# kcat/openal-soft

Measured on AMD Instinct MI355X. Metric: mixed voices/sec @48kHz 1024-sample update, HRTF stereo; fraction of HBM roofline, higher is better.
Workload: dtype f32

## Files before the change

include/oalgpu.h:

```cpp
#ifndef OALGPU_H
#define OALGPU_H

#include <stddef.h>
#include <stdint.h>

#ifdef __cplusplus
extern "C" {
#endif
#if defined(__GNUC__)
#pragma GCC visibility push(default)
#endif

#define OALGPU_BUFFER_LINE_SIZE 1024
#define OALGPU_MAX_RESAMPLER_PADDING 48
#define OALGPU_MAX_RESAMPLER_EDGE 24
#define OALGPU_HRTF_HISTORY_LENGTH 64
#define OALGPU_HRIR_LENGTH 128
#define OALGPU_MAX_SENDS 6
#define OALGPU_MAX_OUTPUT_CHANNELS 32
#define OALGPU_MAX_AMBI_CHANNELS 25
#define OALGPU_MIXER_FRAC_BITS 16

typedef enum oalgpu_error {
    OALGPU_OK = 0,
// ... 176 lines not shown
typedef struct oalgpu_voice_pan {
    float dir[3];
    float spread;
    float dry_gain;
    float send_gain[OALGPU_MAX_SENDS];
} oalgpu_voice_pan;
int oalgpu_context_set_ambi_map(oalgpu_context *ctx, const uint8_t *index, const float *scale);
int oalgpu_slot_set_ambi_map(oalgpu_context *ctx, uint32_t slot, const uint8_t *index, const float *scale);
int oalgpu_voice_set_pan(oalgpu_context *ctx, const uint32_t *voices, const oalgpu_voice_pan *pans, size_t count);

int oalgpu_buffer_queue_link(oalgpu_context *ctx, int buffer, int next_buffer);
int oalgpu_voice_init_queue(oalgpu_context *ctx, uint32_t voice, int first_buffer, int looping, int32_t position,
    uint32_t position_frac);
int oalgpu_voice_queue_state(oalgpu_context *ctx, uint32_t voice, int32_t *current_buffer, uint32_t *buffers_done);
int oalgpu_voice_queue_unqueue(oalgpu_context *ctx, uint32_t voice, uint32_t count);

typedef int32_t (*oalgpu_callback_fn)(void *userptr, void *data, int32_t num_bytes);
int oalgpu_voice_init_callback(oalgpu_context *ctx, uint32_t voice, int fmt_type, uint32_t position_frac,
    oalgpu_callback_fn fn, void *userptr);
typedef struct oalgpu_callback_state {
    int32_t position;
    uint32_t position_frac, num_blocks, block_offset;
    int32_t stopped, play_state, has_buffer;
} oalgpu_callback_state;
int oalgpu_voice_callback_state(oalgpu_context *ctx, uint32_t voice, oalgpu_callback_state *out);

enum oalgpu_adpcm_type { OALGPU_ADPCM_IMA4 = 0, OALGPU_ADPCM_MS = 1 };
int oalgpu_buffer_register_adpcm(oalgpu_context *ctx, const void *data, int adpcm_type, uint32_t channels,
    uint32_t samples_per_block, uint32_t sample_len, uint32_t loop_start, uint32_t loop_end);

int oalgpu_voice_set_start_delay(oalgpu_context *ctx, uint32_t voice, uint32_t samples);

int oalgpu_voice_set_params(oalgpu_context *ctx, const uint32_t *voices,
    const oalgpu_voice_params *params, size_t count);
typedef struct oalgpu_param_block oalgpu_param_block;
int  oalgpu_param_block_create(oalgpu_context *ctx, const uint32_t *voices,
    const oalgpu_voice_params *params, size_t count, oalgpu_param_block **out);
int  oalgpu_param_block_apply(oalgpu_context *ctx, oalgpu_param_block *block);
int  oalgpu_mix_update_run(oalgpu_context *ctx, oalgpu_param_block *const *param_blocks, uint32_t count,
    uint32_t samples_to_do, int post_process);
void oalgpu_param_block_destroy(oalgpu_param_block *block);
int oalgpu_voice_set_state(oalgpu_context *ctx, uint32_t voice, int play_state);

int oalgpu_mix_update(oalgpu_context *ctx, uint32_t samples_to_do, int post_process);
int oalgpu_sync(oalgpu_context *ctx);
typedef struct oalgpu_resident_info {
    int32_t  enabled, failed, running, door_in_device_memory;
    uint32_t launches, updates, parks, timed_launches;
    uint64_t timed_updates;
    double   timed_kernel_ms;
    uint32_t max_updates_per_launch, pad;
    double   wait_door_us, wait_reduction_us, wait_arrival_us, wait_post_us, wait_reduced_us, wait_split_us;
    double   install_us, busy_us, top_us;
} oalgpu_resident_info;
int oalgpu_resident_stats(oalgpu_context *ctx, oalgpu_resident_info *out);
int oalgpu_resident_set_short_run(oalgpu_context *ctx, uint32_t updates);
int oalgpu_resident_set_timing(oalgpu_context *ctx, int enable);
int oalgpu_resident_set_max_updates(oalgpu_context *ctx, uint32_t max_updates);
int oalgpu_set_stream(oalgpu_context *ctx, void *hip_stream);

int oalgpu_read_dry(oalgpu_context *ctx, float *out);
int oalgpu_read_wet(oalgpu_context *ctx, uint32_t slot, float *out);
int oalgpu_read_hrtf_accum(oalgpu_context *ctx, float *out);
int oalgpu_set_bformat_decoder(oalgpu_context *ctx, uint32_t num_out, const float *coeffs_hf,
    const float *coeffs_lf, float xover_norm);
enum oalgpu_output_type {
    OALGPU_OUT_I8 = 0, OALGPU_OUT_U8, OALGPU_OUT_I16, OALGPU_OUT_U16, OALGPU_OUT_I32, OALGPU_OUT_U32, OALGPU_OUT_F32
};
int oalgpu_set_output(oalgpu_context *ctx, int sample_type, float dither_depth, uint32_t dither_seed);
int oalgpu_read_output(oalgpu_context *ctx, void *out, uint32_t samples_to_do, uint32_t frame_step);
enum {
    OALGPU_LIMITER_AUTO_KNEE = 1u << 0, OALGPU_LIMITER_AUTO_ATTACK = 1u << 1, OALGPU_LIMITER_AUTO_RELEASE = 1u << 2,
    OALGPU_LIMITER_AUTO_POST_GAIN = 1u << 3, OALGPU_LIMITER_AUTO_DECLIP = 1u << 4
};
typedef struct oalgpu_limiter_params {
    uint32_t num_channels;
    float sample_rate;
    uint32_t auto_flags;
    float look_ahead_time, hold_time, pre_gain_db, post_gain_db, threshold_db, ratio, knee_db, attack_time, release_time;
} oalgpu_limiter_params;
int oalgpu_limiter_device_params(uint32_t sample_rate, int sample_type, float dither_depth, oalgpu_limiter_params *out);
uint32_t oalgpu_limiter_look_ahead(const oalgpu_limiter_params *params);
int oalgpu_set_output_limiter(oalgpu_context *ctx, const oalgpu_limiter_params *params);
enum oalgpu_uhj_quality { OALGPU_UHJ_IIR = 0, OALGPU_UHJ_FIR256, OALGPU_UHJ_FIR512 };
uint32_t oalgpu_uhj_encoder_delay(int quality);
int oalgpu_set_uhj_encoder(oalgpu_context *ctx, int quality);
enum oalgpu_tsme_quality { OALGPU_TSME_IIR = 0, OALGPU_TSME_FIR256, OALGPU_TSME_FIR512 };
uint32_t oalgpu_tsme_encoder_delay(int quality);
int oalgpu_set_tsme_encoder(oalgpu_context *ctx, int quality);
enum { OALGPU_BS2B_LOW = 1, OALGPU_BS2B_MIDDLE, OALGPU_BS2B_HIGH,
       OALGPU_BS2B_LOW_EASY, OALGPU_BS2B_MIDDLE_EASY, OALGPU_BS2B_HIGH_EASY };
int oalgpu_crossfeed_constants(int level, uint32_t sample_rate, float out[5]);
int oalgpu_set_crossfeed(oalgpu_context *ctx, int level, uint32_t left, uint32_t right);
typedef struct oalgpu_stabilizer_params {
    uint32_t left, right, center;
    float    xover_norm;
} oalgpu_stabilizer_params;
int oalgpu_front_stabilizer_constants(float xover_norm, float *out);
int oalgpu_set_front_stabilizer(oalgpu_context *ctx, const oalgpu_stabilizer_params *params);
int oalgpu_distance_comp_from_distances(uint32_t sample_rate, const float *distances, uint32_t n,
                                        uint32_t *delays, float *gains);
int oalgpu_set_distance_comp(oalgpu_context *ctx, uint32_t n, const uint32_t *delays, const float *gains);

int oalgpu_bus_device_ptr(oalgpu_context *ctx, void **ptr, size_t *nfloats, void **hip_stream);
int oalgpu_mix_voices(oalgpu_context *ctx, uint32_t samples_to_do);
int oalgpu_post_process(oalgpu_context *ctx, uint32_t samples_to_do);
// ... 188 lines not shown
```

openal-soft_amd/csrc/api.hip:

```cpp
#include "api_context.hpp"
namespace oalgpu {

thread_local std::string gLastError;

int Fail(int code, const std::string &msg)
{
    gLastError = msg;
    return code;
}

void ParkResidentContexts(int device);

int UseDevice(int device)
{
    int count = 0;
    if(hipGetDeviceCount(&count) != hipSuccess || count <= 0)
        return Fail(OALGPU_ERR_NO_DEVICE, "no HIP device available (the product has no CPU path)");
    if(device < 0 || device >= count) return Fail(OALGPU_ERR_INVALID, "device ordinal out of range");
    HIP_TRY(hipSetDevice(device));
    ParkResidentContexts(device);
    return OALGPU_OK;
}

}
// ... 927 lines not shown

int oalgpu_slot_set_effect(oalgpu_context *c, uint32_t slot, oalgpu_effect *fx)
{
    if(!c || slot >= c->L.numSlots) return Fail(OALGPU_ERR_INVALID, "oalgpu_slot_set_effect: bad slot");
    if(fx && (EffectOutLines(fx) > c->L.numDry + c->L.numReal || EffectInChannels(fx) > c->L.wetChannels))
        return Fail(OALGPU_ERR_INVALID, "oalgpu_slot_set_effect: the effect's lines do not fit the context's buses");
    if(int rc = oalgpu_sync(c)) return rc;
    c->slotEffect[slot] = fx;
    return OALGPU_OK;
}

int oalgpu_slot_set_reverb(oalgpu_context *c, uint32_t slot, oalgpu_reverb *rev)
{
    if(!c || slot >= c->L.numSlots) return Fail(OALGPU_ERR_INVALID, "oalgpu_slot_set_reverb: bad slot");
    if(rev && c->L.wetChannels < 4)
        return Fail(OALGPU_ERR_INVALID, "oalgpu_slot_set_reverb: the reverb reads a 4-line B-Format wet bus");
    if(rev && ReverbOutLines(rev) > c->L.numDry)
        return Fail(OALGPU_ERR_INVALID, "oalgpu_slot_set_reverb: the effect mixes into more lines than the context has dry lines");
    if(int rc = oalgpu_sync(c)) return rc;
    if(rev) { if(int rc = oalgpu_reverb_set_math_mode(rev, c->exact ? OALGPU_MATH_EXACT : OALGPU_MATH_FAST)) return rc; }
    c->slotReverb[slot] = rev;
    return RebalanceWaveGroups(c);
}

const char *oalgpu_voice_kernel_name(oalgpu_context *c)
{
    if(!c) return "";
    if(c->useWave) return WaveKernelName(c->L);
    return c->exact ? "VoiceMixKernel<true, LINES>" : "VoiceMixKernel<false, LINES>";
}

int oalgpu_resident_stats(oalgpu_context *c, oalgpu_resident_info *out)
{
    if(!c || !out) return Fail(OALGPU_ERR_INVALID, "null argument");
    auto &R = c->res;
    uint32_t w[kRcCount * 16] = {};
    if(R.ready && !R.running)
    {
        if(int rc = UseDevice(c->desc.device)) return rc;
        HIP_TRY(hipMemcpy(w, R.counters.p, sizeof(w), hipMemcpyDeviceToHost));
    }
    std::lock_guard<std::mutex> g(gResLock);
    out->enabled = R.enabled ? 1 : 0; out->failed = R.failed ? 1 : 0; out->running = R.running ? 1 : 0;
    out->door_in_device_memory = R.doorInBar ? 1 : 0;
    out->launches = R.launches; out->updates = R.next; out->parks = uint32_t(R.parks);
    out->timed_launches = uint32_t(R.kernelLaunches); out->timed_updates = R.kernelUpdates; out->timed_kernel_ms = R.kernelMs;
    out->max_updates_per_launch = R.maxUpdates; out->pad = 0;
    const double tick = 0.01, groups = double(std::max<uint32_t>((c->L.numGroups + 127u) / 128u, 1u));
    out->wait_door_us = w[16 * kRcWaitDoor] * tick / groups; out->wait_reduction_us = w[16 * kRcWaitRed] * tick / groups;
    out->wait_arrival_us = w[16 * kRcWaitArrive] * tick; out->wait_post_us = w[16 * kRcWaitPost] * tick;
    out->wait_reduced_us = w[16 * kRcWaitRedDone] * tick; out->wait_split_us = w[16 * kRcWaitSplit] * tick;
    out->install_us = w[16 * kRcInstall] * tick / groups; out->busy_us = w[16 * kRcBusy] * tick / groups;
    out->top_us = w[16 * kRcTop] * tick / groups;
    return OALGPU_OK;
}

int oalgpu_resident_set_short_run(oalgpu_context *c, uint32_t updates)
{
    if(!c) return Fail(OALGPU_ERR_INVALID, "null argument");
    if(int rc = UseCtx(c)) return rc;
    c->res.shortRun = updates;
    c->res.shortRuns = 0; c->res.cooldown = 0;
    return OALGPU_OK;
}

int oalgpu_resident_set_timing(oalgpu_context *c, int enable)
{
    if(!c) return Fail(OALGPU_ERR_INVALID, "null argument");
    if(int rc = UseCtx(c)) return rc;
    c->res.timeLaunches = enable != 0;
    return OALGPU_OK;
}

int oalgpu_resident_set_max_updates(oalgpu_context *c, uint32_t max_updates)
{
    if(!c || max_updates == 0 || max_updates > 0x10000000u) return Fail(OALGPU_ERR_INVALID, "oalgpu_resident_set_max_updates: 1 .. 2^28");
    if(int rc = UseCtx(c)) return rc;
    c->res.maxUpdates = max_updates;
    return OALGPU_OK;
}

int oalgpu_set_carry_accum(oalgpu_context *c, int enable)
{
    if(int rc = BeginSetter(c, "oalgpu_set_carry_accum")) return rc;
    c->carryAccum = enable != 0;
    return OALGPU_OK;
}
```

openal-soft_amd/csrc/kernels.hpp:

```cpp
#pragma once
#include <hip/hip_runtime.h>
#include <stdint.h>

#include "dev_hrtf.hpp"
#include "dev_mix.hpp"
#include "dev_resample.hpp"
#include "dev_voice.hpp"
#include "../host/limiter_params.hpp"
#include "../host/uhj_params.hpp"
#include "../host/stabilizer_params.hpp"
#include "../host/crossfeed_params.hpp"

namespace oalgpu {

enum VoiceFlagBits : uint32_t {
    kFlagFading = 1u << 0,
    kFlagHasHrtf = 1u << 1,
    kFlagDirectFilter = 1u << 2,
    kFlagHrtfDirty = 1u << 3,
    kFlagAmbiScale = 1u << 4,
    kFlagNfc = 1u << 5,
    kFlagQueue = 1u << 7,
    kFlagDelayed = 1u << 6,
    kFlagSendFilterShift = 8
// ... 124 lines not shown
            | (r.keepHrtf ? uint32_t(kFlagHrtfDirty) : 0u));
        ctl.flags = keep | (r.flags & ~(kFlagFading | kFlagHasHrtf | kFlagHrtfDirty | kFlagAmbiScale | kFlagNfc | kFlagDelayed | kFlagQueue))
            | (L.hrtf ? (kFlagHasHrtf | (r.keepHrtf ? 0u : uint32_t(kFlagHrtfDirty))) : 0u);
        for(int i = 0; i < 6; ++i) ctl.sendSlot[i] = (uint32_t(i) < L.numSends) ? r.sendSlot[i] : -1;
        if(L.hrtf && !r.keepHrtf)
        {
            ctl.hrtfTgtDelay[0] = r.hrtfDelay[0]; ctl.hrtfTgtDelay[1] = r.hrtfDelay[1];
            ctl.hrtfTgtGain = r.hrtfGain;
        }
    }
    if(lane == 1) BiquadSetTarget(L.dfilt[size_t{v} * 2 + 0].f, r.dirLp);
    if(lane == 2) BiquadSetTarget(L.dfilt[size_t{v} * 2 + 1].f, r.dirHp);
    if(lane >= 8 && lane < 8 + 2 * L.numSends)
    {
        const uint32_t i = (lane - 8) >> 1, hp = (lane - 8) & 1u;
        BiquadSetTarget(L.sfilt[(size_t{v} * L.numSends + i) * 2 + hp].f, hp ? r.sendHp[i] : r.sendLp[i]);
    }
    if(L.hrtf) { if(!r.keepHrtf) ApplyHrtfTargetWave(L, v, r.hrtfIdx, r.hrtfW, r.hrtfPass, lane); }
    else if(lane < L.numDry)
        L.gainTgt[size_t{v} * L.numDry + lane] = r.dryGains[lane];
    for(uint32_t k = lane; k < L.numSends * L.wetChannels; k += 64)
        L.sendTgt[size_t{v} * L.numSends * L.wetChannels + k] = r.sendGains[k / L.wetChannels][k % L.wetChannels];
}

struct VoiceInitRecord { uint32_t voice; int32_t buffer, looping, position; uint32_t positionFrac; int32_t queue; };

constexpr uint32_t kResidentSets = 4;
constexpr uint32_t kResidentSlots = 16;
constexpr uint32_t kResidentDepth = 8;
constexpr unsigned long long kResidentWatchdogTicks = 200000000ull;

struct ResidentSlot { unsigned long long recs, map, rows; uint32_t samples, pad; };
struct alignas(64) ResidentDoor {
    uint32_t seq;
    uint32_t exitSeq[4];
    uint32_t pad[11];
    ResidentSlot slot[kResidentSlots];
};
enum ResidentCounter : uint32_t {
    kRcArrive0 = 0,
    kRcRedRead = 4,
    kRcRedDone = 5,
    kRcPostDone = 6,
    kRcStarted = 7,
    kRcWaitDoor = 8,
    kRcWaitRed = 9,
    kRcWaitArrive = 10,
    kRcWaitPost = 11,
    kRcWaitRedDone = 12,
    kRcWaitSplit = 13,
    kRcInstall = 14,
    kRcBusy = 15,
    kRcTop = 16,
    kRcCount = 17
};
enum ResidentHostFlag : uint32_t { kRhResident = 0, kRhError = 1, kRhProgress = 2,
    kRhFault = 3,
    kRhCount = 4 };
struct ResidentArgs {
    const ResidentDoor *door;
    uint32_t *counters;
    uint32_t *hostFlags;
    float *partBase;
    uint32_t setStride;
    uint32_t base, endSeq;
    uint32_t redPerUpdate;
    uint32_t startedTarget, launchId;
};

void LaunchResample(hipStream_t s, bool exact, const ResampleSpec &spec, const float *src, uint32_t frac,
    uint32_t increment, float *dst, uint32_t n);
void LaunchMix(hipStream_t s, const float *in, uint32_t n, float *out, uint32_t nlines, float *cur,
    const float *tgt, uint32_t counter, uint32_t outpos);
void LaunchMixHrtf(hipStream_t s, bool exact, const float *in, float *accum, uint32_t irsize, const float *coeffs,
    uint32_t dL, uint32_t dR, float gain, float step, const float *oldcoeffs, uint32_t odL, uint32_t odR,
    float oldgain, int blend, uint32_t n);
void LaunchMixDirectHrtf(hipStream_t s, bool exact, float *left, float *right, const float *in, uint32_t nch,
    float *accum, SplitterState *splitters, const float *hfscales, const float *chanCoeffs, uint32_t irsize,
    uint32_t n, float *temp);
void LaunchBiquadDual(hipStream_t s, BiquadState *f0, BiquadState *f1, const float *src, float *dst, uint32_t n);
void LaunchGetCoeffs(hipStream_t s, const HrtfStoreDev &st, const float *dirs, uint32_t count, float *coeffs,
    uint32_t *delays);

void LaunchPostDirectHrtfFast(hipStream_t s, float *left, float *right, const float *in, uint32_t nch, float *accum,
    SplitterState *splitters, const float *hfscales, const float *chanCoeffs, uint32_t irsize, uint32_t n, float *temp,
    hipEvent_t evDone = nullptr);

inline uint32_t ReducePostReduceGroups(const DeviceLayout &L) { return uint32_t((BusFloats(L) + 63u) / 64u); }
void LaunchReducePostFused(hipStream_t s, const DeviceLayout &L, const float *carry, float *left, float *right, const float *in, uint32_t nch,
    const float *accIn, float *carryOut, const SplitterState *spIn, SplitterState *spOut, const float *hfscales, const float *chanCoeffs,
    uint32_t irsize, uint32_t n, float *xf, uint32_t *arrived, uint32_t epoch, const float runPower[4], hipEvent_t evDone,
    float *hostOut, uint32_t *hostFlag, uint32_t hostSeq, uint32_t *outArrived, uint32_t outTarget, uint32_t *reduced, uint32_t reducedEpoch);
void LaunchPostDirectHrtfFused(hipStream_t s, float *left, float *right, const float *in, uint32_t nch, const float *accIn, float *carryOut,
    const SplitterState *spIn, SplitterState *spOut, const float *hfscales, const float *chanCoeffs, uint32_t irsize, uint32_t n,
    float *xf, uint32_t *arrived, uint32_t epoch, const float runPower[4], hipEvent_t evDone = nullptr,
    float *hostOut = nullptr, uint32_t *hostFlag = nullptr, uint32_t hostSeq = 0, uint32_t *outArrived = nullptr, uint32_t outTarget = 0);
void LaunchBusReduceResident(hipStream_t s, const DeviceLayout &L, const float *carry, uint32_t *counters, uint32_t *hostFlags, uint32_t set,
    uint32_t arriveTarget, uint32_t postDoneTarget);
uint32_t PostResidentFirGroups();
void LaunchPostResident(hipStream_t s, float *left, float *right, const float *in, uint32_t nch, const float *accIn, float *carryOut,
    const SplitterState *spIn, SplitterState *spOut, const float *hfscales, const float *chanCoeffs, uint32_t irsize, uint32_t n,
    float *xf, uint32_t *arrived, uint32_t epoch, const float runPower[4], hipEvent_t evDone, float *hostOut, uint32_t *hostFlag, uint32_t hostSeq,
    uint32_t *counters, uint32_t *hostFlags, uint32_t redDoneTarget, uint32_t postDoneTarget, uint32_t progressValue);

void LaunchBFormatDecode(hipStream_t s, bool exact, float *out, const float *lines, SplitterState *states, float *bands,
    const float *gainsHf, const float *gainsLf, uint32_t nin, uint32_t nout, uint32_t n);
void LaunchDither(hipStream_t s, float *lines, uint32_t nlines, uint32_t n, float quantScale, uint32_t seed);
// ... 155 lines not shown
```

openal-soft_amd/csrc/voice_wave16.hip:

```cpp
#define OALGPU_WAVE_NO_LAUNCHER
#include "voice_wave.hip"

#pragma clang fp contract(off)

namespace oalgpu {
namespace {

constexpr int kW16Outs = kLine / 64;

constexpr int kW16Rd = 1184;
constexpr int kW16Rd2 = kMaxEdge + kPre * 64 + 8;
constexpr int kW16Area = kResampleDataSize + kLine;
static_assert(kW16Rd % 64 == 32 && kW16Rd >= kMaxPad + kPre * 64 + 8, "rd2 sits half the banks away from rd");
static_assert(kW16Rd + kW16Rd2 <= kW16Area, "the twice-parked window fits");
static_assert(kResampleDataSize >= kLine + 64, "a send's filter scan parks the unfiltered samples in the window's area");
constexpr int kW16DumpF2 = 64 * 17 + 68;
static_assert(kW16DumpF2 * 2 <= kW16Area, "the dump fits");
struct W16PhaseB {
    uint32_t xh[2][kXhDw];
    uint32_t hr[2][kHrDw];
    uint32_t hro[2][kHrDw];
    float in0[2 * kHist];
};
static_assert(sizeof(W16PhaseB) <= size_t(kW16Area) * 4, "phase B fits the area (nothing of it is written before the sample line is back in registers)");
// ... 104 lines not shown
            A[s][c] = __builtin_bit_cast(h8, q);
        }
#pragma unroll
    for(int T = 0; T < TILES; ++T)
    {
        __builtin_amdgcn_sched_barrier(0);
        const uint32_t j = (T == 4 && i > 3u) ? 3u : i;
        h8 B[2][3];
#pragma unroll
        for(int s = 0; s < 2; ++s)
        {
            const u4 *p = reinterpret_cast<const u4*>(xh[s]) + 32 * T + 2u * j + g;
#pragma unroll
            for(int c = 0; c < 3; ++c) B[s][c] = __builtin_bit_cast(h8, p[4 * c]);
        }
        f4 ta = {0.0f, 0.0f, 0.0f, 0.0f}, tb = ta, tc = ta;
#pragma unroll
        for(int c = 0; c < 3; ++c)
        {
            ta = __builtin_amdgcn_mfma_f32_16x16x32_f16(A[1][c], B[0][c], ta, 0, 0, 0);
            tb = __builtin_amdgcn_mfma_f32_16x16x32_f16(A[0][c], B[1][c], tb, 0, 0, 0);
            tc = __builtin_amdgcn_mfma_f32_16x16x32_f16(A[0][c], B[0][c], tc, 0, 0, 0);
        }
        f4 sum = __builtin_elementwise_fma((ta + tb) + tc, vinv, acc[T]);
        asm volatile("" : "+v"(sum));
        if(!LOW8 || i < 8u) acc[T] = sum;
        __builtin_amdgcn_sched_barrier(0);
    }
}

__device__ __forceinline__ float W16ReadLaneF(float v, int l)
{ return __builtin_bit_cast(float, __builtin_amdgcn_readlane(__builtin_bit_cast(int, v), l)); }

__device__ __forceinline__ float W16StageResponse(uint32_t (&hr)[2][kHrDw], float h, uint32_t lane)
{
    float sh, inv;
    HalfScale(WaveMaxBits(__builtin_bit_cast(uint32_t, __builtin_fabsf(h))), sh, inv);
    uint32_t hi, lo;
    SplitHalf2(h * sh, 0.0f, hi, lo);
    uint32_t *hz32 = &hr[0][0];
    for(uint32_t k = lane; k < uint32_t(2 * kHrDw); k += 64) hz32[k] = 0u;
    uint16_t *hz = reinterpret_cast<uint16_t*>(&hr[0][0]);
    const uint32_t u = 80u - lane;
    hz[0 * kHrHalves + u] = uint16_t(hi); hz[1 * kHrHalves + u] = uint16_t(lo);
    return __builtin_bit_cast(float, __builtin_amdgcn_readfirstlane(__builtin_bit_cast(int, inv)));
}

__device__ __forceinline__ uint32_t W16VoiceOf(uint32_t group, uint32_t wave, uint32_t waves)
{
    const uint32_t a = wave >> 2, b = wave & 3u;
    return group * waves + 4u * a + ((a + b) & 3u);
}

struct Next16 { const ParamRecord *recs; const int32_t *map; const float *rows; ResidentArgs res; };
struct W16Sends {
    BiquadSlot *sfilt; const float *sendTgt; float *sendCur; float *streams; uint32_t *lineGains;
    uint32_t numSends, wetCh, lineStride, spv;
};

template<bool PROF, int WAVES, bool SENDS = false, bool RES = false>
__global__ void OALGPU_SINGLE_DS_OPS __launch_bounds__(WAVES * 64) VoiceWave16Kernel(WaveArgsHrtf L, uint32_t samplesToDo, Next16 next, WaveProf prof, W16Sends S)
{
    unsigned long long tEntry = 0;
    if constexpr (PROF) tEntry = __builtin_readcyclecounter();
    constexpr uint32_t kW16Waves = uint32_t(WAVES), kW16Threads = uint32_t(WAVES) * 64u;
    __shared__ W16Wg<WAVES> sm;
    const uint32_t t = threadIdx.x;
    uint32_t lane = t & 63u;
    const uint32_t wave = __builtin_amdgcn_readfirstlane(t >> 6);
    const uint32_t group = blockIdx.x;
    const uint32_t irStride = L.irStride;
    uint32_t N = samplesToDo;
    W16Lds &w = sm.w[wave];
    asm volatile("; argument block resident" :: "s"(L.tables), "s"(L.buffers), "s"(L.ctl), "s"(L.prev), "s"(L.dfilt), "s"(L.hrtfOld),
        "s"(L.hrtfTgt), "s"(L.hist), "s"(L.ambi), "s"(L.startDelay), "s"(L.queueDone), "s"(L.partHrtf), "s"(L.hrirs),
        "s"(next.recs), "s"(next.map), "s"(L.numVoices), "s"(L.irStride), "s"(L.pad), "s"(samplesToDo));

    const uint32_t vRaw = W16VoiceOf(group, wave, kW16Waves);
    const bool haveVoice = vRaw < L.numVoices;
    const uint32_t lastVoice = L.numVoices - 1u;
    const uint32_t v = haveVoice ? vRaw : lastVoice;
    const uint32_t keyVoice = group * uint32_t(kW16Waves);

    uint32_t upd = 0u, updBase = 0u;
    if constexpr (RES)
    {
        const ResidentArgs &RA = next.res;
        upd = updBase = RA.base;
        if(t == 0)
        {
            const uint32_t old = __hip_atomic_fetch_add(RA.counters + 16u * kRcStarted, 1u, __ATOMIC_RELAXED, __HIP_MEMORY_SCOPE_AGENT);
            if(old + 1u == RA.startedTarget)
                __hip_atomic_store(RA.hostFlags + 16u * kRhResident, RA.launchId, __ATOMIC_RELAXED, __HIP_MEMORY_SCOPE_SYSTEM);
        }
    }
    for(;;)
    {
    uint32_t tU = threadIdx.x;
    if constexpr (RES) { asm volatile("" : "+v"(tU)); lane = tU & 63u; }
    const uint32_t t = tU;
    if constexpr (RES)
    {
        const ResidentArgs &RA = next.res;
        if(t == 0)
        {
            const unsigned long long tTop = __builtin_amdgcn_s_memrealtime();
            uint32_t go = 0u, fault = 0u;
            unsigned long long recs = 0ull, map = 0ull, rowsP = 0ull;
            uint32_t smp = 0u;
            if(upd != RA.endSeq)
            {
                const ResidentDoor *door = RA.door;
                const uint32_t *exitp = &door->exitSeq[RA.launchId & 3u];
                const uint32_t *rr = RA.counters + 16u * kRcRedRead;
                const bool needRed = int32_t(upd - kResidentSets) >= 0;
                const uint32_t want = (upd - kResidentSets + 1u) * RA.redPerUpdate;
                unsigned long long t0 = 0ull;
                uint32_t waitedFor = 0u;
                for(uint32_t spins = 0;; ++spins)
                {
                    const uint32_t ex = ResLoadSys(exitp), sq = ResLoadSys(&door->seq), rd = needRed ? ResLoadDev(rr) : want;
                    if(int32_t(ex - upd) <= 0) break;
                    const bool rung = int32_t(sq - upd) > 0, redOk = int32_t(rd - want) >= 0;
                    if(rung && redOk) { go = 1u; break; }
                    if(spins == 0u) { t0 = __builtin_amdgcn_s_memrealtime(); waitedFor = rung ? 2u : 1u; }
                    else if((spins & 15u) == 15u && __builtin_amdgcn_s_memrealtime() - t0 > kResidentWatchdogTicks)
                    {
                        fault = 1u;
                        uint32_t *fi = RA.hostFlags + 16u * kRhFault;
                        fi[0] = upd; fi[1] = sq; fi[2] = ex; fi[3] = rd; fi[4] = want; fi[5] = group; fi[6] = RA.launchId;
                        fi[7] = uint32_t(__builtin_amdgcn_s_memrealtime() - t0);
                        break;
                    }
                    if(spins < 32u) __builtin_amdgcn_s_sleep(2); else __builtin_amdgcn_s_sleep(24);
                }
                if(waitedFor && (group & 127u) == 0u)
                    __hip_atomic_fetch_add(RA.counters + 16u * (waitedFor == 1u ? kRcWaitDoor : kRcWaitRed), uint32_t(__builtin_amdgcn_s_memrealtime() - t0),
                        __ATOMIC_RELAXED, __HIP_MEMORY_SCOPE_AGENT);
                if(go)
                {
                    const ResidentSlot *sl = &door->slot[upd % kResidentSlots];
                    recs = ResLoadSys(&sl->recs); map = ResLoadSys(&sl->map); rowsP = ResLoadSys(&sl->rows); smp = ResLoadSys(&sl->samples);
                }
            }
            if(fault) __hip_atomic_store(RA.hostFlags + 16u * kRhError, 1u, __ATOMIC_RELAXED, __HIP_MEMORY_SCOPE_SYSTEM);
            if((group & 127u) == 0u)
                __hip_atomic_fetch_add(RA.counters + 16u * kRcTop, uint32_t(__builtin_amdgcn_s_memrealtime() - tTop), __ATOMIC_RELAXED, __HIP_MEMORY_SCOPE_AGENT);
            sm.res[0] = go; sm.res[1] = smp;
// ... 26 lines not shown
    auto stamp = [&](int slot)
    {
        if constexpr (PROF) { if(prof.times && haveVoice && (t & 63u) == 0u) prof.times[size_t{v} * 8 + slot] = __builtin_readcyclecounter(); }
    };
    if constexpr (PROF) { if(prof.times && haveVoice && (t & 63u) == 0u) prof.times[size_t{v} * 8 + 0] = tEntry; }
    auto stamp2 = [&](int slot)
    {
        if constexpr (PROF) { if(prof.times && haveVoice && (t & 63u) == 0u) prof.times[size_t{L.numVoices} * 8 + size_t{v} * 8 + slot] = __builtin_readcyclecounter(); }
    };
    const VoiceHead head = LoadHeadScalar(L.ctl + v);
    const BufferItem buf = LoadCtlBufferScalar(L.ctl + v);
    const VoiceTail tail = LoadTailScalar(L.ctl + v);
    asm volatile("" ::: "memory");
    const VoiceHead headK = LoadHeadScalar(L.ctl + (keyVoice < L.numVoices ? keyVoice : lastVoice));
    asm volatile("" ::: "memory");
    const int psK = headK.playState, kK = headK.rsKind;
    const uint32_t mK = kK == 2 ? 4u : headK.rsM, lK = kK == 2 ? 1u : headK.rsL, offK = headK.rsFilterOffset;

    const bool eligK = keyVoice < L.numVoices && (kK == 2 || (kK == 3 && (mK == 12 || mK == 24)))
        && (psK == OALGPU_VOICE_PLAYING || psK == OALGPU_VOICE_STOPPING);
    bool stageRows = true;
    if constexpr (RES) { if(upd != updBase) stageRows = !(eligK && sm.tabKey == offK * 8u + uint32_t(kK) && sm.tabM == mK); }
    if constexpr (RES) __syncthreads();
    if(eligK && stageRows)
    {
        typedef const __attribute__((address_space(1))) void *gvoidp;
        typedef __attribute__((address_space(3))) void *lvoidp;
        const float *src = L.tables + offK + size_t{lane >> 1} * (2u * mK) + (lane & 1u);
        for(uint32_t pp = wave; pp < mK / 2u; pp += uint32_t(kW16Waves))
        {
            __builtin_amdgcn_global_load_lds((gvoidp)(src + 2u * pp), (lvoidp)&sm.tabF[32u * pp], 4, 0, 0);
            __builtin_amdgcn_global_load_lds((gvoidp)(src + mK + 2u * pp), (lvoidp)&sm.tabP[32u * pp], 4, 0, 0);
        }
        if(t == 0) { sm.tabKey = offK * 8u + uint32_t(kK); sm.tabM = mK; sm.tabL = lK; }
    }

    const int vstate = head.playState;
    const bool mixes = haveVoice && (vstate == OALGPU_VOICE_PLAYING || vstate == OALGPU_VOICE_STOPPING);
    const bool playing = haveVoice && vstate == OALGPU_VOICE_PLAYING;
    bool active = mixes && head.step >= 1u;
    const bool dirty = (head.flags & kFlagHrtfDirty) != 0;
    SrcPlan plan = PlanSource(head, N);
    bool looping = false;
    if(head.curBuffer >= 0)
    {
        looping = head.loopBuffer >= 0 && ((head.flags & kFlagQueue) || !(head.position >= 0 && uint32_t(head.position) >= buf.loopEnd));
        plan.prefetch = plan.prefetch && GatherCovers(plan.bsrc, buf, looping, uint32_t(head.position));
    }
    if(head.flags & (kFlagDelayed | kFlagQueue)) plan.prefetch = false;
    const uint32_t sM = head.rsKind == 2 ? 4u : head.rsM, sL = head.rsKind == 2 ? 1u : head.rsL;
    const bool regPath = active && plan.prefetch && eligK && (head.rsKind == 2 || head.rsKind == 3)
        && head.rsFilterOffset * 8u + uint32_t(head.rsKind) == offK * 8u + uint32_t(kK) && sM == mK
        && !(head.step == kFracOne && head.positionFrac == 0u);
    float pre[kPre];
#pragma unroll
    for(int i = 0; i < kPre; ++i) pre[i] = 0.0f;
    float prevv = 0.0f;
    if(regPath)
    {
        GatherStatic(pre, plan.bsrc, buf, looping, uint32_t(head.position), lane);
        prevv = (lane < kMaxPad) ? L.prev[size_t{v} * kMaxPad + lane] : 0.0f;
    }

    if(!eligK)
    {
        if(wave == 0)
        {
            const uint32_t cand = keyVoice + lane;
            bool eligible = false;
            uint32_t off = 0, m = 0, l = 0;
            int kind = 0;
            if(lane < uint32_t(kW16Waves) && cand < L.numVoices)
            {
                const VoiceCtl &c = L.ctl[cand];
                kind = c.rsKind; off = c.rsFilterOffset; m = c.rsM; l = c.rsL;
                if(kind == 2) { m = 4; l = 1; }
                eligible = (kind == 2 || (kind == 3 && (m == 12 || m == 24)))
                    && (c.playState == OALGPU_VOICE_PLAYING || c.playState == OALGPU_VOICE_STOPPING);
            }
            const unsigned long long mask = __ballot(eligible);
            if(mask)
            {
                const int firstLane = __ffsll((long long)mask) - 1;
                const uint32_t key = uint32_t(__shfl(int(off * 8u + uint32_t(kind)), firstLane));
                const uint32_t fm = uint32_t(__shfl(int(m), firstLane)), fl = uint32_t(__shfl(int(l), firstLane));
                if(lane == 0) { sm.tabKey = key; sm.tabM = fm; sm.tabL = fl; }
            }
            else if(lane == 0) { sm.tabKey = 0xffffffffu; sm.tabM = 0; sm.tabL = 0; }
        }
        __syncthreads();
        const uint32_t key = sm.tabKey, m = sm.tabM;
        if(key != 0xffffffffu)
        {
            const float *filter = L.tables + (key >> 3);
            for(uint32_t idx = t; idx < (m / 2u) * 32u; idx += uint32_t(kW16Threads))
            {
                const uint32_t p = idx >> 5, pi = idx & 31u;
                const float *row = filter + pi * 2u * m;
                sm.tabF[idx] = f2{row[2u * p], row[2u * p + 1u]};
                sm.tabP[idx] = f2{row[m + 2u * p], row[m + 2u * p + 1u]};
            }
        }
    }
    if(regPath)
    {
        const bool isShort = buf.fmt == OALGPU_FMT_SHORT;
        if(lane < kMaxPad) { w.a.rd[lane] = prevv; if(lane) w.a.rd2[lane - 1u] = prevv; }
#pragma unroll
        for(int i = 0; i < kPre; ++i)
        {
            const float sv = GatherDecode(pre[i], isShort);
            w.a.rd[kMaxEdge + lane + 64u * uint32_t(i)] = sv;
            w.a.rd2[kMaxEdge - 1u + lane + 64u * uint32_t(i)] = sv;
        }
    }
    asm volatile("s_waitcnt vmcnt(0)" ::: "memory");
    __syncthreads();
    stamp(7);
    __builtin_amdgcn_s_setprio(2);

    uint32_t outPos = 0;
    if(mixes && !active && !playing && lane == 0) L.ctl[v].playState = OALGPU_VOICE_STOPPED;
    if(active && (head.flags & kFlagDelayed))
    {
        const uint32_t d = L.startDelay[v];
        if(!playing)
        {
            if(lane == 0) { L.ctl[v].playState = OALGPU_VOICE_STOPPED; L.ctl[v].flags = head.flags & ~kFlagDelayed; L.startDelay[v] = 0u; }
            active = false;
        }
        else if(d >= N) { if(lane == 0) L.startDelay[v] = d - N; active = false; }
        else
        {
            outPos = d;
            if(lane == 0) L.startDelay[v] = 0u;
            for(uint32_t k = lane; k < outPos; k += 64) w.g.smp[k] = 0.0f;
        }
    }

    f4 accM[2][5];
#pragma unroll
    for(int e = 0; e < 2; ++e)
#pragma unroll
        for(int b = 0; b < 5; ++b) accM[e][b] = f4{0.0f, 0.0f, 0.0f, 0.0f};

    uint32_t counter = 0, fademix = 0, todo = 0;
    float endGain = 0.0f, gainAfterBlend = 0.0f;
    float fstv = 0.0f, histv = 0.0f;
    f2 hT = {0.0f, 0.0f};
    int32_t bufferItem = head.curBuffer;
    if constexpr (SENDS)
    {
        if(haveVoice && !active && lane < S.spv)
            S.lineGains[(size_t{v} * S.spv + lane) * LineBlockDwords(S.lineStride) + 3u * S.lineStride] = 0u;
    }
    if(active)
    {
        float outs[kW16Outs];
        if(regPath)
        {
            WaveSync();
            const float *rdb = w.a.rd + (kMaxEdge - sL), *rd2b = w.a.rd2 + (kMaxEdge - sL);
            const uint32_t rdbIndex = uint32_t(kMaxEdge) - sL;
            if(sM == 24u) ResampleRingRegs<24, true>(sm.tabF, sm.tabP, rdb, head.positionFrac, head.step, N, outs, lane, rd2b, rdbIndex);
            else if(sM == 12u) ResampleRingRegs<12, true>(sm.tabF, sm.tabP, rdb, head.positionFrac, head.step, N, outs, lane, rd2b, rdbIndex);
            else ResampleRingRegs<4, false>(sm.tabF, sm.tabP, rdb, head.positionFrac, head.step, N, outs, lane, nullptr, 0u);
            asm volatile("" : "+v"(lane));
            if(playing)
            {
                const uint32_t srcOffset = uint32_t((uint64_t{N} * head.step + head.positionFrac) >> kFracBits);
                if(lane < kMaxPad) L.prev[size_t{v} * kMaxPad + lane] = w.a.rd[srcOffset + lane];
            }
        }
        else
        {
            W16GenView gv{w.g.rd, w.g.smp - kHist, nullptr, w.best, w.pad};
            LoadResampledWave<true, false>(sm, gv, L, v, lane, head, playing, N - outPos, N - outPos, bufferItem, looping,
                SrcPlan{false, plan.bdst, plan.bsrc}, outPos);
            asm volatile("" : "+v"(lane));
            WaveSync();
#pragma unroll
            for(int j = 0; j < kW16Outs; ++j) outs[j] = w.g.smp[lane + 64u * uint32_t(j)];
        }
        if(N < uint32_t(kLine))
        {
#pragma unroll
            for(int j = 0; j < kW16Outs; ++j) if(lane + 64u * uint32_t(j) >= N) outs[j] = 0.0f;
        }
        stamp(1);
        __builtin_amdgcn_s_setprio(1);
        fstv = (lane < 32u) ? reinterpret_cast<const float*>(L.dfilt + size_t{v} * 2)[lane] : 0.0f;
        histv = L.hist[size_t{v} * kHist + lane];
// ... 229 lines not shown
                __builtin_fabsf(endGain));
            HalfScale(__builtin_bit_cast(uint32_t, mxw * gmax), sx, invX);
            invX = __builtin_bit_cast(float, __builtin_amdgcn_readfirstlane(__builtin_bit_cast(int, invX)));
            sx = __builtin_bit_cast(float, __builtin_amdgcn_readfirstlane(__builtin_bit_cast(int, sx)));
        }
        const float step64 = mainStep * 64.0f * sx;
        auto buildEar = [&](uint32_t d, auto fullTag)
        {
            constexpr bool FULL = decltype(fullTag)::value;
            if(lane < 32u) { w.b.xh[0][lane] = 0u; w.b.xh[1][lane] = 0u; }
            for(uint32_t dw = 32u + (N >> 1) + lane; dw < uint32_t(kXhDw); dw += 64u) { w.b.xh[0][dw] = 0u; w.b.xh[1][dw] = 0u; }
            WaveSync();
            uint16_t *xz = reinterpret_cast<uint16_t*>(&w.b.xh[0][0]) + 64u + lane + d;
            if(lane < d)
            {
                const float headP = (lane < N) ? w.b.in0[kHist - d + lane] * gainAt(lane, true) : 0.0f;
                uint32_t hi, lo;
                SplitHalf2(headP * sx, 0.0f, hi, lo);
                uint16_t *xh0 = reinterpret_cast<uint16_t*>(&w.b.xh[0][0]) + 64u + lane;
                xh0[0] = uint16_t(hi); xh0[kXhHalves] = uint16_t(lo);
            }
            const uint32_t i00 = lane + d;
            const float g0s = gainAt(i00, true) * sx;
            const float gls = __builtin_fmaf(mainStep, float(i00), gbase) * sx;
#pragma unroll
            for(int j = 0; j < kW16Outs; j += 2)
            {
                const float ga = (j == 0) ? g0s : __builtin_fmaf(step64, float(j), gls);
                const float gb = __builtin_fmaf(step64, float(j + 1), gls);
                float p0 = outs[j] * ga, p1 = outs[j + 1] * gb;
                if(!FULL || j + 2 == kW16Outs)
                {
                    if(i00 + 64u * uint32_t(j) >= N) p0 = 0.0f;
                    if(i00 + 64u * uint32_t(j + 1) >= N) p1 = 0.0f;
                }
                uint32_t hi, lo;
                SplitHalf2(p0, p1, hi, lo);
                xz[64 * j] = uint16_t(hi); xz[kXhHalves + 64 * j] = uint16_t(lo);
                xz[64 * (j + 1)] = uint16_t(hi >> 16); xz[kXhHalves + 64 * (j + 1)] = uint16_t(lo >> 16);
            }
        };

#pragma unroll
        for(int e = 0; e < 2; ++e)
        {
            const uint32_t d = tail.tgtDelay[e];
            if(N == uint32_t(kLine)) buildEar(d, std::true_type{}); else buildEar(d, std::false_type{});
            uint16_t *xz = reinterpret_cast<uint16_t*>(&w.b.xh[0][0]);
            if(e == 0) stamp2(1);
            const float invH = W16StageResponse(w.b.hr, e == 0 ? hT.x : hT.y, lane);
            WaveSync();
            if(e == 0) stamp2(2);
            FirMfmaEar<5, false>(accM[e], w.b.xh, w.b.hr, invX * invH, lane);
            if(e == 0) stamp2(3);
            if(oldPass)
            {
                const uint32_t od = tail.oldDelay[e];
                float xo = 0.0f;
                if(lane < fademix) xo = w.b.in0[kHist - od + lane] * (oldStep * float(fademix - lane));
                float sxo, invXo;
                HalfScale(WaveMaxBits(__builtin_bit_cast(uint32_t, __builtin_fabsf(xo))), sxo, invXo);
                invXo = __builtin_bit_cast(float, __builtin_amdgcn_readfirstlane(__builtin_bit_cast(int, invXo)));
                uint32_t hi, lo;
                SplitHalf2(xo * sxo, 0.0f, hi, lo);
                WaveSync();
                xz[0 * kXhHalves + 64u + lane] = uint16_t(hi); xz[1 * kXhHalves + 64u + lane] = uint16_t(lo);
                if(lane < 40u) { w.b.xh[0][64u + lane] = 0u; w.b.xh[1][64u + lane] = 0u; }
                const float invHO = W16StageResponse(w.b.hro, e == 0 ? hO.x : hO.y, lane);
                WaveSync();
                FirMfmaEar<1, true>(accM[e], w.b.xh, w.b.hro, invXo * invHO, lane);
            }
            WaveSync();
            stamp(3 + e);
        }
    }

    if(active)
    {
        if(dirty && (counter == 0 || fademix))
        {
            if(lane < irStride) reinterpret_cast<f2*>(L.hrtfOld + size_t{v} * irStride * 2)[lane] = hT;
        }
        if(lane == 0)
        {
            VoiceCtl &c = L.ctl[v];
            if(counter == 0 || fademix) { c.hrtfOldDelay[0] = tail.tgtDelay[0]; c.hrtfOldDelay[1] = tail.tgtDelay[1]; }
            c.hrtfOldGain = todo ? endGain : gainAfterBlend;
            uint32_t flags = (head.flags | kFlagFading) & ~kFlagDelayed;
            if(counter == 0 || fademix) flags &= ~kFlagHrtfDirty;
            c.flags = flags;
            if(!playing) c.playState = OALGPU_VOICE_STOPPED;
            else
            {
                int32_t bufPosInt = head.position;
                uint32_t bufPosFrac = head.positionFrac + head.step * (N - outPos);
                const uint32_t samplesDone = bufPosFrac >> kFracBits;
                bufPosInt = AddSat(bufPosInt, int32_t(samplesDone));
                bufPosFrac &= kFracMask;
                if(bufferItem >= 0 && bufPosInt > 0 && (head.flags & kFlagQueue))
                {
                    uint32_t buffersDone = 0;
                    const int32_t before = bufferItem;
                    AdvanceQueue(L.buffers, bufferItem, head.loopBuffer, bufPosInt, buffersDone);
                    if(buffersDone) L.queueDone[v] += buffersDone;
                    if(bufferItem >= 0 && bufferItem != before) c.buf = L.buffers[bufferItem];
                }
// ... 151 lines not shown
```

openal-soft_amd/oalgpu/__init__.py:

```python
import ctypes as C
import os

import numpy as np

PKG_DIR = os.path.dirname(os.path.dirname(os.path.abspath(__file__)))
LIB_PATH = os.path.join(PKG_DIR, "liboalgpu.so")

BUFFER_LINE = 1024
MAX_PAD = 48
HRTF_HIST = 64
HRIR_LEN = 128
MAX_SENDS = 6
(OUT_I8, OUT_U8, OUT_I16, OUT_U16, OUT_I32, OUT_U32, OUT_F32) = range(7)
MAX_OUT = 32
MAX_AMBI = 25
MATH_EXACT, MATH_FAST = 0, 1
(RS_POINT, RS_LINEAR, RS_SPLINE, RS_GAUSSIAN, RS_FAST_BSINC12, RS_BSINC12, RS_FAST_BSINC24,
 RS_BSINC24, RS_FAST_BSINC48, RS_BSINC48) = range(10)
FMT_UBYTE, FMT_SHORT, FMT_INT, FMT_FLOAT, FMT_DOUBLE, FMT_MULAW, FMT_ALAW = range(7)
FMT_DTYPES = {FMT_UBYTE: np.uint8, FMT_SHORT: np.int16, FMT_INT: np.int32, FMT_FLOAT: np.float32,
              FMT_DOUBLE: np.float64, FMT_MULAW: np.uint8, FMT_ALAW: np.uint8}
VOICE_STOPPED, VOICE_PLAYING, VOICE_STOPPING, VOICE_PENDING = range(4)

f32p = C.POINTER(C.c_float)
# ... 681 lines not shown
    def set_front_stabilizer(self, left, right=None, center=None, xover_norm=5000.0 / 48000.0):
        lib.oalgpu_set_front_stabilizer.argtypes = [C.c_void_p, C.POINTER(StabilizerParams)]
        if left is None:
            check(lib.oalgpu_set_front_stabilizer(self.h, None), "oalgpu_set_front_stabilizer")
            return
        params = StabilizerParams(left, right, center, xover_norm)
        check(lib.oalgpu_set_front_stabilizer(self.h, C.byref(params)), "oalgpu_set_front_stabilizer")

    def set_distance_comp(self, delays, gains=None):
        u32p = C.POINTER(C.c_uint32)
        lib.oalgpu_set_distance_comp.argtypes = [C.c_void_p, C.c_uint32, u32p, f32p]
        if delays is None:
            check(lib.oalgpu_set_distance_comp(self.h, 0, None, None), "oalgpu_set_distance_comp")
            return
        d = np.ascontiguousarray(delays, np.uint32)
        g = np.ascontiguousarray(gains, np.float32)
        assert d.ndim == 1 and d.shape == g.shape
        check(lib.oalgpu_set_distance_comp(self.h, d.size, d.ctypes.data_as(u32p), _fp(g)), "oalgpu_set_distance_comp")

    def read_output(self, samples_to_do=BUFFER_LINE, frame_step=2):
        lib.oalgpu_read_output.argtypes = [C.c_void_p, C.c_void_p, C.c_uint32, C.c_uint32]
        dt = [np.int8, np.uint8, np.int16, np.uint16, np.int32, np.uint32, np.float32][getattr(self, "_out_type", 6)]
        out = np.zeros(samples_to_do * frame_step, dt)
        check(lib.oalgpu_read_output(self.h, out.ctypes.data_as(C.c_void_p), samples_to_do, frame_step), "oalgpu_read_output")
        return out

    def set_slot_convolution(self, slot, conv):
        lib.oalgpu_slot_set_convolution.argtypes = [C.c_void_p, C.c_uint32, C.c_void_p]
        check(lib.oalgpu_slot_set_convolution(self.h, slot, conv.h if conv is not None else None))

    def set_slot_effect(self, slot, fx):
        lib.oalgpu_slot_set_effect.argtypes = [C.c_void_p, C.c_uint32, C.c_void_p]
        check(lib.oalgpu_slot_set_effect(self.h, slot, fx.h if fx is not None else None), "oalgpu_slot_set_effect")

    def set_slot_reverb(self, slot, rev):
        lib.oalgpu_slot_set_reverb.argtypes = [C.c_void_p, C.c_uint32, C.c_void_p]
        check(lib.oalgpu_slot_set_reverb(self.h, slot, rev.h if rev is not None else None))

    def mix(self, samples_to_do=BUFFER_LINE, post_process=False):
        check(lib.oalgpu_mix_update(self.h, samples_to_do, 1 if post_process else 0),
              "oalgpu_mix_update")

    def sync(self):
        check(lib.oalgpu_sync(self.h), "oalgpu_sync")

    def resident_stats(self):
        class Info(C.Structure):
            _fields_ = [("enabled", C.c_int32), ("failed", C.c_int32), ("running", C.c_int32), ("door_in_device_memory", C.c_int32),
                        ("launches", C.c_uint32), ("updates", C.c_uint32), ("parks", C.c_uint32), ("timed_launches", C.c_uint32),
                        ("timed_updates", C.c_uint64), ("timed_kernel_ms", C.c_double),
                        ("max_updates_per_launch", C.c_uint32), ("pad", C.c_uint32),
                        ("wait_door_us", C.c_double), ("wait_reduction_us", C.c_double), ("wait_arrival_us", C.c_double),
                        ("wait_post_us", C.c_double), ("wait_reduced_us", C.c_double), ("wait_split_us", C.c_double),
                        ("install_us", C.c_double), ("busy_us", C.c_double), ("top_us", C.c_double)]
        info = Info()
        lib.oalgpu_resident_stats.argtypes = [C.c_void_p, C.POINTER(Info)]
        check(lib.oalgpu_resident_stats(self.h, C.byref(info)), "oalgpu_resident_stats")
        return {k: getattr(info, k) for k, _ in Info._fields_ if k != "pad"}

    def resident_set_short_run(self, updates):
        lib.oalgpu_resident_set_short_run.argtypes = [C.c_void_p, C.c_uint32]
        check(lib.oalgpu_resident_set_short_run(self.h, updates), "oalgpu_resident_set_short_run")

    def resident_set_timing(self, on):
        lib.oalgpu_resident_set_timing.argtypes = [C.c_void_p, C.c_int]
        check(lib.oalgpu_resident_set_timing(self.h, 1 if on else 0), "oalgpu_resident_set_timing")

    def resident_set_max_updates(self, n):
        lib.oalgpu_resident_set_max_updates.argtypes = [C.c_void_p, C.c_uint32]
        check(lib.oalgpu_resident_set_max_updates(self.h, n), "oalgpu_resident_set_max_updates")

    def dry(self):
        n = self.desc.num_dry_channels + self.desc.num_real_channels
        out = np.zeros((n, BUFFER_LINE), np.float32)
        check(lib.oalgpu_read_dry(self.h, _fp(out)), "oalgpu_read_dry")
        return out

    def wet(self, slot):
        out = np.zeros((self.desc.wet_channels, BUFFER_LINE), np.float32)
        check(lib.oalgpu_read_wet(self.h, slot, _fp(out)), "oalgpu_read_wet")
        return out

    def hrtf_accum(self):
        out = np.zeros((BUFFER_LINE + HRIR_LEN, 2), np.float32)
        check(lib.oalgpu_read_hrtf_accum(self.h, _fp(out)), "oalgpu_read_hrtf_accum")
        return out

    def voice_state(self, voice):
        st = VoiceState()
        check(lib.oalgpu_voice_readback(self.h, voice, C.byref(st)), "oalgpu_voice_readback")
        return st

    def bus_device_ptr(self):
        p, n, s = C.c_void_p(), C.c_size_t(), C.c_void_p()
        check(lib.oalgpu_bus_device_ptr(self.h, C.byref(p), C.byref(n), C.byref(s)))
        return p.value, n.value, s.value

    def voice_kernel_name(self):
        lib.oalgpu_voice_kernel_name.restype = C.c_char_p
        lib.oalgpu_voice_kernel_name.argtypes = [C.c_void_p]
        return lib.oalgpu_voice_kernel_name(self.h).decode()

    def set_timing(self, enable=True):
        check(lib.oalgpu_set_timing(self.h, 1 if enable else 0))

    def last_update_ms(self):
        a, b = C.c_float(), C.c_float()
# ... 234 lines not shown
```

Baseline: 114.6 million.

## Prefetch next update's source window during HRTF FIR in resident kernel

In the resident (persistent) kernel, the register-held source window (pre[]) and the resampler history are now gathered for the next update while the current update's second-ear MFMA FIR runs. A per-lane key over the buffer, position and loop state validates the prefetched data at the next iteration. On a match the gather at update start is skipped, otherwise it falls back to the normal gather. A timing counter (window_us) is added to the stats. The cost is extra registers kept live across iterations, which may reduce occupancy, and wasted loads whenever the prediction misses.

```diff
diff --git a/include/oalgpu.h b/include/oalgpu.h
--- a/include/oalgpu.h
+++ b/include/oalgpu.h
@@ -252,6 +252,7 @@
     uint32_t max_updates_per_launch, pad;
     double   wait_door_us, wait_reduction_us, wait_arrival_us, wait_post_us, wait_reduced_us, wait_split_us;
     double   install_us, busy_us, top_us;
+    double   window_us;
 } oalgpu_resident_info;
 int oalgpu_resident_stats(oalgpu_context *ctx, oalgpu_resident_info *out);
 int oalgpu_resident_set_short_run(oalgpu_context *ctx, uint32_t updates);
diff --git a/openal-soft_amd/csrc/api.hip b/openal-soft_amd/csrc/api.hip
--- a/openal-soft_amd/csrc/api.hip
+++ b/openal-soft_amd/csrc/api.hip
@@ -1003,6 +1003,7 @@
     out->wait_reduced_us = w[16 * kRcWaitRedDone] * tick; out->wait_split_us = w[16 * kRcWaitSplit] * tick;
     out->install_us = w[16 * kRcInstall] * tick / groups; out->busy_us = w[16 * kRcBusy] * tick / groups;
     out->top_us = w[16 * kRcTop] * tick / groups;
+    out->window_us = w[16 * kRcWindow] * tick / groups;
     return OALGPU_OK;
 }
 
diff --git a/openal-soft_amd/csrc/kernels.hpp b/openal-soft_amd/csrc/kernels.hpp
--- a/openal-soft_amd/csrc/kernels.hpp
+++ b/openal-soft_amd/csrc/kernels.hpp
@@ -200,7 +200,8 @@
     kRcInstall = 14,
     kRcBusy = 15,
     kRcTop = 16,
-    kRcCount = 17
+    kRcWindow = 17,
+    kRcCount = 18
 };
 enum ResidentHostFlag : uint32_t { kRhResident = 0, kRhError = 1, kRhProgress = 2,
     kRhFault = 3,
diff --git a/openal-soft_amd/csrc/voice_wave16.hip b/openal-soft_amd/csrc/voice_wave16.hip
--- a/openal-soft_amd/csrc/voice_wave16.hip
+++ b/openal-soft_amd/csrc/voice_wave16.hip
@@ -180,6 +180,33 @@
     return group * waves + 4u * a + ((a + b) & 3u);
 }
 
+constexpr uint32_t kW16NoWindow = 0xffffffffu;
+__device__ __forceinline__ uint32_t W16WindowKey(const BufferItem &b, int32_t curBuffer, uint32_t position, bool looping, uint32_t lane)
+{
+    const uint64_t d = uint64_t(uintptr_t(b.data));
+    uint32_t k = 0u;
+    k = lane == 0u ? uint32_t(d) : k;
+    k = lane == 1u ? uint32_t(d >> 32) : k;
+    k = lane == 2u ? uint32_t(b.fmt) : k;
+    k = lane == 3u ? b.frameStep : k;
+    k = lane == 4u ? b.sampleLen : k;
+    k = lane == 5u ? b.loopStart : k;
+    k = lane == 6u ? b.loopEnd : k;
+    k = lane == 7u ? uint32_t(b.next) : k;
+    k = lane == 8u ? uint32_t(curBuffer) : k;
+    k = lane == 9u ? position : k;
+    k = lane == 10u ? (looping ? 1u : 0u) : k;
+    return k;
+}
+__device__ __forceinline__ uint32_t W16WindowCount(const BufferItem &b, bool looping, uint32_t position)
+{
+    const uint32_t whole = uint32_t(kPre) * 64u;
+    if(!looping) return whole;
+    if(position >= b.loopEnd) return 0u;
+    const uint64_t reach = uint64_t{b.loopEnd - position} + (b.loopEnd - b.loopStart);
+    return reach < whole ? uint32_t(reach) : whole;
+}
+
 struct Next16 { const ParamRecord *recs; const int32_t *map; const float *rows; ResidentArgs res; };
 struct W16Sends {
     BiquadSlot *sfilt; const float *sendTgt; float *sendCur; float *streams; uint32_t *lineGains;
@@ -222,6 +249,14 @@
                 __hip_atomic_store(RA.hostFlags + 16u * kRhResident, RA.launchId, __ATOMIC_RELAXED, __HIP_MEMORY_SCOPE_SYSTEM);
         }
     }
+    float pre[kPre];
+    float prePrev = 0.0f;
+    uint32_t preKey = kW16NoWindow;
+    if constexpr (RES)
+    {
+#pragma unroll
+        for(int i = 0; i < kPre; ++i) pre[i] = 0.0f;
+    }
     for(;;)
     {
     uint32_t tU = threadIdx.x;
@@ -354,15 +389,28 @@
     const bool regPath = active && plan.prefetch && eligK && (head.rsKind == 2 || head.rsKind == 3)
         && head.rsFilterOffset * 8u + uint32_t(head.rsKind) == offK * 8u + uint32_t(kK) && sM == mK
         && !(head.step == kFracOne && head.positionFrac == 0u);
-    float pre[kPre];
-#pragma unroll
-    for(int i = 0; i < kPre; ++i) pre[i] = 0.0f;
+    if constexpr (!RES)
+    {
+#pragma unroll
+        for(int i = 0; i < kPre; ++i) pre[i] = 0.0f;
+    }
     float prevv = 0.0f;
     if(regPath)
     {
-        GatherStatic(pre, plan.bsrc, buf, looping, uint32_t(head.position), lane);
-        prevv = (lane < kMaxPad) ? L.prev[size_t{v} * kMaxPad + lane] : 0.0f;
-    }
+        bool requested = false;
+        if constexpr (RES)
+        {
+            const uint32_t now = W16WindowKey(buf, head.curBuffer, uint32_t(head.position), looping, lane);
+            requested = __ballot(now != preKey) == 0ull && plan.bsrc <= W16WindowCount(buf, looping, uint32_t(head.position));
+        }
+        if(!requested)
+        {
+            GatherStatic(pre, plan.bsrc, buf, looping, uint32_t(head.position), lane);
+            prevv = (lane < kMaxPad) ? L.prev[size_t{v} * kMaxPad + lane] : 0.0f;
+        }
+        else prevv = prePrev;
+    }
+    preKey = kW16NoWindow;
 
     if(!eligK)
     {
@@ -416,8 +464,19 @@
             w.a.rd2[kMaxEdge - 1u + lane + 64u * uint32_t(i)] = sv;
         }
     }
+    if constexpr (RES)
+    {
+#pragma unroll
+        for(int i = 0; i < kPre; ++i) pre[i] = 0.0f;
+        prePrev = 0.0f;
+    }
     asm volatile("s_waitcnt vmcnt(0)" ::: "memory");
     __syncthreads();
+    if constexpr (RES)
+    {
+        if(t == 0 && (group & 127u) == 0u)
+            __hip_atomic_fetch_add(next.res.counters + 16u * kRcWindow, uint32_t(__builtin_amdgcn_s_memrealtime()) - sm.res[6], __ATOMIC_RELAXED, __HIP_MEMORY_SCOPE_AGENT);
+    }
     stamp(7);
     __builtin_amdgcn_s_setprio(2);
 
@@ -440,6 +499,37 @@
         }
     }
 
+    auto requestAhead = [&]()
+    {
+        if constexpr (RES)
+        {
+            if(regPath && playing)
+            {
+                const uint32_t fracEnd = head.positionFrac + head.step * N;
+                int32_t pos = AddSat(head.position, int32_t(fracEnd >> kFracBits));
+                bool ends = false;
+                if(pos > 0)
+                {
+                    if(looping)
+                    {
+                        if(uint32_t(pos) >= buf.loopEnd) pos = int32_t(((uint32_t(pos) - buf.loopStart) % (buf.loopEnd - buf.loopStart)) + buf.loopStart);
+                    }
+                    else if(uint32_t(pos) >= buf.sampleLen) ends = true;
+                }
+                const bool loopingN = head.loopBuffer >= 0 && !(pos >= 0 && uint32_t(pos) >= buf.loopEnd);
+                const uint32_t cnt = (ends || pos < 0) ? 0u : W16WindowCount(buf, loopingN, uint32_t(pos));
+                if(cnt)
+                {
+                    __builtin_amdgcn_sched_barrier(0);
+                    uint32_t laneQ = lane;
+                    asm volatile("" : "+v"(laneQ));
+                    GatherStatic(pre, cnt, buf, loopingN, uint32_t(pos), laneQ);
+                    prePrev = (laneQ < kMaxPad) ? L.prev[size_t{v} * kMaxPad + laneQ] : 0.0f;
+                    preKey = W16WindowKey(buf, head.curBuffer, uint32_t(pos), loopingN, lane);
+                }
+            }
+        }
+    };
     f4 accM[2][5];
 #pragma unroll
     for(int e = 0; e < 2; ++e)
@@ -775,6 +865,7 @@
             WaveSync();
             if(e == 0) stamp2(2);
             FirMfmaEar<5, false>(accM[e], w.b.xh, w.b.hr, invX * invH, lane);
+            if(e == 1) requestAhead();
             if(e == 0) stamp2(3);
             if(oldPass)
             {
diff --git a/openal-soft_amd/oalgpu/__init__.py b/openal-soft_amd/oalgpu/__init__.py
--- a/openal-soft_amd/oalgpu/__init__.py
+++ b/openal-soft_amd/oalgpu/__init__.py
@@ -757,7 +757,7 @@
                         ("max_updates_per_launch", C.c_uint32), ("pad", C.c_uint32),
                         ("wait_door_us", C.c_double), ("wait_reduction_us", C.c_double), ("wait_arrival_us", C.c_double),
                         ("wait_post_us", C.c_double), ("wait_reduced_us", C.c_double), ("wait_split_us", C.c_double),
-                        ("install_us", C.c_double), ("busy_us", C.c_double), ("top_us", C.c_double)]
+                        ("install_us", C.c_double), ("busy_us", C.c_double), ("top_us", C.c_double), ("window_us", C.c_double)]
         info = Info()
         lib.oalgpu_resident_stats.argtypes = [C.c_void_p, C.POINTER(Info)]
         check(lib.oalgpu_resident_stats(self.h, C.byref(info)), "oalgpu_resident_stats")
```

After: 112.6 million. 1.7% lower.
